# RaduAlexandru/permuto_sdf

Hardware: AMD Instinct MI355X
Metric: ray-samples/sec (encode+MLP+composite) (higher is better)
Workload: dtype f32 (MLP products on 2 fp16 operand pieces per fp32 value, fp32 accumulation; the 3-piece / 24-bit figure is value_fp32_equivalent_24bit)

## Files before the change

### include/psdf.h

```cpp
#ifndef PSDF_H
#define PSDF_H
#include <stdint.h>
#ifdef __cplusplus
extern "C" {
#endif

int64_t psdf_encode_convention(int which);
int psdf_encode_set_conventions(uint32_t hash_multiplier, int rank_tie_raises_later);

int psdf_encode_set_forward_pairs(int pairs);

int psdf_encode_forward(int pos_dim, int nr_feat, int64_t N, int nr_levels, int capacity, const float* positions,
    const float* lattice, const float* scale_factor, const float* shifts, const float* window, int concat_points,
    float points_scaling, float* sliced, void* stream);

int psdf_encode_forward_mark(int pos_dim, int nr_feat, int64_t N, int nr_levels, int capacity, const float* positions,
    const float* lattice, const float* scale_factor, const float* shifts, const float* window, int concat_points,
    float points_scaling, float* sliced, unsigned char* touched_blocks, int block_rows_log2, void* stream);

int psdf_encode_backward(int pos_dim, int nr_feat, int64_t N, int nr_levels, int capacity, const float* positions,
    const float* lattice, const float* scale_factor, const float* shifts, const float* window, int concat_points,
    float points_scaling, const float* grad_sliced, float* grad_lattice, float* grad_positions, void* stream);

int64_t psdf_encode_backward_workspace_bytes(int pos_dim, int nr_feat, int64_t N, int nr_levels, int capacity);
int psdf_encode_backward_ws(int pos_dim, int nr_feat, int64_t N, int nr_levels, int capacity, const float* positions,
    const float* lattice, const float* scale_factor, const float* shifts, const float* window, int concat_points,
    float points_scaling, const float* grad_sliced, float* grad_lattice, float* grad_positions, void* workspace,
    int64_t workspace_bytes, void* stream);
int psdf_encode_backward_level_shares(int* counts, int max_levels);


int psdf_encode_double_backward(int pos_dim, int nr_feat, int64_t N, int nr_levels, int capacity, const float*
    positions, const float* lattice, const float* scale_factor, const float* shifts, const float* window, int
    concat_points, float points_scaling, const float* dd_positions, const float* grad_sliced, float* grad_lattice,
    float* grad_grad_sliced, void* stream);
int psdf_encode_double_backward_ws(int pos_dim, int nr_feat, int64_t N, int nr_levels, int capacity, const float* positions,
                                   const float* lattice, const float* scale_factor, const float* shifts, const float* window,
                                   int concat_points, float points_scaling, const float* dd_positions, const float* grad_sliced,
                                   float* grad_lattice, float* grad_grad_sliced, const float* grad_sliced_direct,
                                   void* workspace, int64_t workspace_bytes, void* stream);

int psdf_mlp_pack_f16(int n_layers, const int* dims, const float* const* weights, const float* const* biases, float* packed,
    void* stream);
int psdf_mlp_forward_f16(int n_layers, const int* dims, int64_t N, const float* X, const float* packed, float* Y, void* stream);

int psdf_mlp_forward_set_form(int waves);
int psdf_mlp_forward_last_form(void);

int psdf_neus_composite_forward(int nr_rays, const int* start_end, int equal, int fixed, int max_nr_samples, const float* sdf,
    const float* dirs, const float* gradients, const float* dt, const float* rgb, const float* inv_s, float cos_anneal_ratio,
    float* pred, float* bg, float* weights, void* stream);
int psdf_neus_composite_backward(int nr_rays, const int* start_end, int equal, int fixed, int max_nr_samples, int max_per_ray,
    const float* grad_pred, const float* grad_bg, const float* sdf, const float* dirs, const float* gradients, const float* dt,
    const float* rgb, const float* inv_s, float cos_anneal_ratio, int reference_compat, float* grad_sdf, float* grad_gradients,
    float* grad_rgb, float* grad_inv_s, void* stream);

int psdf_nerf_composite_forward(int nr_rays, const int* start_end, int equal, int fixed, int max_nr_samples, const float* raw_density,
                                const float* dt, const float* rgb, const float* fg_pred, const float* fg_bg, float* pred_bg,
                                float* pred, void* stream);
int psdf_nerf_composite_backward(int nr_rays, const int* start_end, int equal, int fixed, int max_nr_samples, int max_per_ray,
                                 const float* grad_pred, const float* fg_bg, const float* raw_density, const float* dt,
                                 const float* rgb, int reference_compat, float* grad_raw_density, float* grad_rgb,
// ... 302 lines not shown
```

### permuto_sdf_amd/csrc/encode.hip

```cpp
#include <cstdio>
#include <cstring>
#include <mutex>
#include <type_traits>
#include <vector>

#include "encode_device.h"
#include "encode_plan.h"

namespace {

struct FwdArgs {
  int64_t N;
  int L;
  uint32_t capacity;
  EncConv conv;
  const float *lattice, *scale_factor, *shifts, *window;
  float points_scaling;
  int pad_points;
  float* sliced;
  unsigned char* touched;
  int touch_shift, blocks_per_level;
};

template <int P, int F>
// ... 241 lines not shown
    for (int i = threadIdx.x; i < SC_SLOTS; i += blockDim.x) {
      const uint32_t row = tags[i];
      if (row != SC_EMPTY) {
#pragma unroll
        for (int f = 0; f < F; f++) {
          const float v = sums[i * F + f];
          if (v != 0.f) atomicAdd(table_grad + (int64_t)row * F + f, v);
        }
      }
    }
  }
  static constexpr size_t bytes() { return (size_t)(SC_SLOTS + SC_SLOTS * F + 4) * 4; }
};

template <typename SC>
__device__ __forceinline__ bool cache_vote(SC& sc, int hits, int tries) {
  hits = (int)psdf::wave_sum((float)hits);
  tries = (int)psdf::wave_sum((float)tries);
  if (psdf::lane_id() == 0) {
    atomicAdd(&sc.stats[0], hits);
    atomicAdd(&sc.stats[1], tries);
  }
  __syncthreads();
  return sc.stats[0] * 8 >= sc.stats[1];
}

struct Queues {
  uint16_t* rows;
  float* vals;
  int* tails;
  int cap, np, shift;
};
using psdf::enc_plan::Q_MAX_PARTS;
constexpr int Q_LDS_INTS = 4 * Q_MAX_PARTS + 4;

struct LevelQueues {
  char* rows;
  char* vals;
  uint32_t mask;
};
template <int F>
__device__ __forceinline__ LevelQueues level_queues(const Queues& Q, int level) {
  const int64_t e = (int64_t)level * Q.np * Q.cap;
  return LevelQueues{reinterpret_cast<char*>(Q.rows + e), reinterpret_cast<char*>(Q.vals + e * F), (1u << Q.shift) - 1u};
}
template <int F>
__device__ __forceinline__ void queue_store(const LevelQueues& LQ, uint32_t o, uint32_t row, const float* v) {
  *reinterpret_cast<uint16_t*>(LQ.rows + (o * 2u)) = (uint16_t)(row & LQ.mask);
  if (F == 2) {
    *reinterpret_cast<float2*>(LQ.vals + (o * 8u)) = make_float2(v[0], v[F - 1]);
  } else {
#pragma unroll
    for (int f = 0; f < F; f++) *reinterpret_cast<float*>(LQ.vals + (o * (uint32_t)(F * 4) + (uint32_t)(f * 4))) = v[f];
  }
}

template <int NC, int F>
__device__ __forceinline__ void queue_push(const Queues& Q, int level, int* q_cnt, int* q_base,
                                           const uint32_t (&crow)[NC], const float (&cval)[NC][F],
                                           float* __restrict__ table_grad) {
  int* q_aux = q_base + Q_MAX_PARTS;
  const LevelQueues LQ = level_queues<F>(Q, level);
  if (threadIdx.x < Q.np) q_cnt[threadIdx.x] = 0;
  __syncthreads();
  int slot[NC];
#pragma unroll
  for (int r = 0; r < NC; r++)
    if (crow[r] != Q_NONE) slot[r] = atomicAdd(&q_cnt[crow[r] >> Q.shift], 1);
  __syncthreads();
  if (threadIdx.x < Q.np) {
    const int c = q_cnt[threadIdx.x];
    const int base = c ? atomicAdd(&Q.tails[level * Q.np + threadIdx.x], c) : 0;
    q_base[threadIdx.x] = base;
    q_aux[threadIdx.x] = (int)threadIdx.x * Q.cap + base;
  }
  __syncthreads();
#pragma unroll
  for (int r = 0; r < NC; r++) {
    if (crow[r] == Q_NONE) continue;
    const int part = crow[r] >> Q.shift;
    const int idx = q_base[part] + slot[r];
    if (idx < Q.cap) {
      queue_store<F>(LQ, (uint32_t)(q_aux[part] + slot[r]), crow[r], cval[r]);
    } else {
#pragma unroll
      for (int f = 0; f < F; f++) atomicAdd(table_grad + (int64_t)crow[r] * F + f, cval[r][f]);
    }
  }
}

template <int NC>
__device__ __forceinline__ void queue_push_staged(const Queues& Q, int level, int* q_cnt, int* q_base, int* q_off, int* q_gd,
                                                  float* stage, const uint32_t (&crow)[NC],
                                                  const float (&cval)[NC][2], float* __restrict__ table_grad) {
  uint32_t* st_row = reinterpret_cast<uint32_t*>(stage);
  float2* st_val = reinterpret_cast<float2*>(stage + NC * PSDF_BLOCK);
  const LevelQueues LQ = level_queues<2>(Q, level);
  if (threadIdx.x < Q.np) q_cnt[threadIdx.x] = 0;
  __syncthreads();
  int slot[NC];
#pragma unroll
  for (int r = 0; r < NC; r++)
    if (crow[r] != Q_NONE) slot[r] = atomicAdd(&q_cnt[crow[r] >> Q.shift], 1);
  __syncthreads();
  if (threadIdx.x < 64) {
    const int lane = threadIdx.x;
    const int c = lane < Q.np ? q_cnt[lane] : 0;
    const int incl = psdf::wave_incl_scan_add_i(c);
    if (lane < Q.np) {
      const int base = c ? atomicAdd(&Q.tails[level * Q.np + lane], c) : 0;
      const int off = incl - c;
      q_off[lane] = off;
      q_base[lane] = base - off;
      q_gd[lane] = lane * Q.cap + base - off;
      if (lane == Q.np - 1) q_off[Q.np] = incl;
    }
  }
  __syncthreads();
#pragma unroll
  for (int r = 0; r < NC; r++)
    if (crow[r] != Q_NONE) {
      const int i = q_off[crow[r] >> Q.shift] + slot[r];
      st_row[i] = crow[r];
      st_val[i] = make_float2(cval[r][0], cval[r][1]);
    }
  __syncthreads();
  const int total = q_off[Q.np];
  for (int i = threadIdx.x; i < total; i += PSDF_BLOCK) {
    const uint32_t row = st_row[i];
    const float2 v = st_val[i];
    const int part = row >> Q.shift;
    const int idx = i + q_base[part];
    if (idx < Q.cap) {
      const float vv[2] = {v.x, v.y};
      queue_store<2>(LQ, (uint32_t)(i + q_gd[part]), row, vv);
    } else {
      atomicAdd(table_grad + (int64_t)row * 2, v.x);
      atomicAdd(table_grad + (int64_t)row * 2 + 1, v.y);
    }
  }
}

template <int F, typename SC>
__device__ __forceinline__ void cache_drain_to_queue(SC& sc, const Queues& Q, int level, int* q_cnt,
                                                     int* q_base, float* __restrict__ table_grad) {
  for (int base = 0; base < SC::SC_SLOTS; base += PSDF_BLOCK) {
    const int i = base + threadIdx.x;
    uint32_t crow[1];
    float cval[1][F];
    const uint32_t tag = sc.tags[i];
    static_assert(SC_EMPTY == Q_NONE, "an empty slot is 'no contribution'");
    crow[0] = tag;
#pragma unroll
    for (int f = 0; f < F; f++) cval[0][f] = sc.sums[i * F + f];
    queue_push<1, F>(Q, level, q_cnt, q_base, crow, cval, table_grad);
    sc.tags[i] = SC_EMPTY;
  }
  __syncthreads();
}

struct LevelPlan {
  int n;
  uint32_t gen;
  uint32_t* times;
  uint16_t first[42];
};
template <int P, int F, bool LATTICE, bool POS, bool QUEUE, bool DBL = false>
#if !defined(PSDF_ENC_QWAVES)
#define PSDF_ENC_QWAVES 5
#endif
__global__ void __launch_bounds__(PSDF_BLOCK, QUEUE ? ((P <= 3 && F == 2) ? PSDF_ENC_QWAVES : 4) : 1)
    encode_bwd_kernel(int64_t N, int L, uint32_t capacity, EncConv conv, const float* __restrict__ positions,
                      const float* __restrict__ lattice, const float* __restrict__ scale_factor,
                      const float* __restrict__ shifts, const float* __restrict__ window, float points_scaling,
                      const float* __restrict__ grad_sliced, float* __restrict__ grad_lattice,
                      float* __restrict__ grad_positions, Queues Q, const float* __restrict__ dd_positions = nullptr,
                      float* __restrict__ grad_grad_sliced = nullptr, int pad_points = 0,
                      const float* __restrict__ grad_sliced2 = nullptr, LevelPlan plan = LevelPlan{}) {
  static_assert(!(DBL && POS), "the double backward has no position output");
  extern __shared__ __align__(16) float lds[];
#if defined(PSDF_ENC_PROFILE)
  const long long psdf_prof_t0 = (long long)wall_clock64();
#endif
  int level = blockIdx.y, bx = blockIdx.x, gx = gridDim.x;
  long long plan_t0 = 0;
  if (plan.n) {
    level = 0;
    for (int l = 1; l < plan.n; l++)
      if ((int)blockIdx.x >= (int)plan.first[l]) level = l;
    bx = (int)blockIdx.x - (int)plan.first[level];
    gx = (int)plan.first[level + 1] - (int)plan.first[level];
    plan_t0 = (long long)wall_clock64();
  }
  auto plan_report = [&]() {
    if (plan.n && plan.times && threadIdx.x == 0) {
      long long dt = (long long)wall_clock64() - plan_t0;
      dt = dt < 1 ? 1 : (dt > 0xFFFFFF ? 0xFFFFFF : dt);
      __hip_atomic_store(plan.times + blockIdx.x, ((plan.gen & 255u) << 24) | (uint32_t)dt, __ATOMIC_RELAXED, __HIP_MEMORY_SCOPE_SYSTEM);
    }
  };
  const int64_t ntiles = (N + PSDF_BLOCK - 1) / PSDF_BLOCK;
  if (level >= L) {
    if (DBL) {
      const int e = level - L;
      for (int64_t tile = bx; tile < ntiles; tile += gx) {
        const int64_t n = tile * PSDF_BLOCK + threadIdx.x;
        if (n >= N) continue;
        float u[P];
        load_pos<P>(dd_positions, n, u);
#pragma unroll
        for (int f = 0; f < F; f++) {
          const int d = e * F + f;
          float v = 0.f;
#pragma unroll
          for (int i = 0; i < P; i++)
            if (i == d) v = u[i] * points_scaling;
          if ((d < P || pad_points) && grad_grad_sliced) grad_grad_sliced[((int64_t)level * F + f) * N + n] = v;
        }
      }
    }
    if (POS) {
      const int e = level - L;
      for (int64_t tile = bx; tile < ntiles; tile += gx) {
        const int64_t n = tile * PSDF_BLOCK + threadIdx.x;
        if (n >= N) continue;
#pragma unroll
        for (int f = 0; f < F; f++) {
          const int d = e * F + f;
          if (d < P)
            atomicAdd(grad_positions + n * P + d, grad_sliced[((int64_t)level * F + f) * N + n] * points_scaling);
        }
      }
    }
    plan_report();
    return;
  }
  if (window[level] == 0.f) {
    if (DBL && grad_grad_sliced) {
      for (int64_t tile = bx; tile < ntiles; tile += gx) {
        const int64_t n = tile * PSDF_BLOCK + threadIdx.x;
        if (n >= N) continue;
#pragma unroll
        for (int f = 0; f < F; f++) grad_grad_sliced[((int64_t)level * F + f) * N + n] = 0.f;
      }
    }
    plan_report();
    return;
  }
  using SCache = ScatterCache<F, QUEUE ? 4096 : 8192>;
  SCache sc;
  int* q_cnt = reinterpret_cast<int*>(lds + SCache::bytes() / 4);
  int* q_base = q_cnt + Q_MAX_PARTS;
  int* q_off = q_base + Q_MAX_PARTS;
  int* q_gd = q_off + Q_MAX_PARTS + 1;
  int* q_vote = q_gd + Q_MAX_PARTS;
  if (QUEUE && threadIdx.x < 3) q_vote[threadIdx.x] = 0;
  if (LATTICE) sc.init(lds);
  bool use_cache = LATTICE;
  int hot = 0;
  int hits = 0, tries = 0, iter = 0;
  const float w = window[level];
  const int64_t tbase = (int64_t)level * capacity * F;
  float sfl[P], shl[P];
#pragma unroll
  for (int i = 0; i < P; i++) {
    sfl[i] = scale_factor[level * P + i];
    shl[i] = shifts[level * P + i];
  }
  constexpr int SPT = QUEUE ? QUEUE_SPT : 1;
  constexpr int NC = SPT * (P + 1);
  const int64_t ntiles_w = (N + (int64_t)PSDF_BLOCK * SPT - 1) / ((int64_t)PSDF_BLOCK * SPT);
  for (int64_t tile = bx; tile < ntiles_w; tile += gx, iter++) {
    uint32_t crow[NC];
    float cval[NC][F];
#pragma unroll
    for (int c = 0; c < NC; c++) {
      crow[c] = Q_NONE;
#pragma unroll
      for (int f = 0; f < F; f++) cval[c][f] = 0.f;
    }
#pragma unroll
    for (int sp = 0; sp < SPT; sp++) {
      const int64_t n = (tile * SPT + sp) * PSDF_BLOCK + threadIdx.x;
      if (n < N) {
        float g[F], g2[F];
#pragma unroll
        for (int f = 0; f < F; f++) {
          g[f] = grad_sliced[((int64_t)level * F + f) * N + n];
          g2[f] = (DBL && grad_sliced2) ? grad_sliced2[((int64_t)level * F + f) * N + n] : 0.f;
        }
        float pos[P];
        load_pos<P>(positions, n, pos);
        Simplex<P> s;
// ... 57 lines not shown
#pragma unroll
            for (int f = 0; f < F; f++) dbary[r] = dbary[r] + lattice[tbase + (int64_t)row * F + f] * w * g[f];
          }
        }
        if (DBL && grad_grad_sliced) {
#pragma unroll
          for (int f = 0; f < F; f++) grad_grad_sliced[((int64_t)level * F + f) * N + n] = gg[f];
        }
        if (POS) {
          dbary[P + 1] = dbary[P + 1] + dbary[0];
          float dE[P + 1];
          const float invp = 1.0f / (P + 1);
#pragma unroll
          for (int i = 0; i <= P; i++) {
            float a = 0.f, b = 0.f;
#pragma unroll
            for (int k = 0; k <= P + 1; k++) {
              if (k == P - s.rank[i]) a = dbary[k];
              if (k == P + 1 - s.rank[i]) b = dbary[k];
            }
            dE[i] = (a - b) * invp;
          }
#pragma unroll
          for (int i = 0; i < P; i++) {
            float acc = 0.f;
#pragma unroll
            for (int j = 0; j <= i; j++) acc = acc + dE[j];
            acc = acc - dE[i + 1] * (float)(i + 1);
            atomicAdd(grad_positions + n * P + i, acc * sfl[i]);
          }
        }
      }
    }
    if (LATTICE) {
#pragma unroll
      for (int c = 0; c < NC; c++) {
        const bool own = combine_runs16<F>(crow[c], cval[c]);
        bool absorbed = false;
        if (own && use_cache) {
          const int rc = sc.add(crow[c], cval[c], hot);
          absorbed = rc != 0;
          hits += (rc == 2);
          tries++;
        }
        if (!own || absorbed) crow[c] = Q_NONE;
      }
    }
    if (LATTICE) {
      if (QUEUE) {
        uint32_t all = Q_NONE;
#pragma unroll
        for (int c = 0; c < NC; c++) all &= crow[c];
        const bool any = all != Q_NONE;
        bool go = !use_cache && iter > 0;
        if (!go) {
          const int vw = iter % 3;
          if (threadIdx.x == 0) q_vote[vw == 2 ? 0 : vw + 1] = 0;
          if (__builtin_amdgcn_ballot_w64(any) != 0ull && psdf::lane_id() == 0) q_vote[vw] = 1;
          __syncthreads();
          go = q_vote[vw] != 0;
        }
        if (go) {
          if constexpr (F == 2 && NC * PSDF_BLOCK * 3 * 4 <= SCache::SC_SLOTS * (1 + F) * 4) {
            if (!use_cache && iter > 0)
              queue_push_staged<NC>(Q, level, q_cnt, q_base, q_off, q_gd, lds, crow, cval, grad_lattice + tbase);
            else
              queue_push<NC, F>(Q, level, q_cnt, q_base, crow, cval, grad_lattice + tbase);
          } else {
            queue_push<NC, F>(Q, level, q_cnt, q_base, crow, cval, grad_lattice + tbase);
          }
        }
      } else {
#pragma unroll
        for (int c = 0; c < NC; c++)
          if (crow[c] != Q_NONE) {
#pragma unroll
            for (int f = 0; f < F; f++) atomicAdd(grad_lattice + tbase + (int64_t)crow[c] * F + f, cval[c][f]);
          }
      }
    }
    if (LATTICE && iter == 0) {
      use_cache = cache_vote(sc, hits, tries);
      if (QUEUE && !use_cache) cache_drain_to_queue<F>(sc, Q, level, q_cnt, q_base, grad_lattice + tbase);
    }
  }
  if (LATTICE && !(QUEUE && !use_cache)) sc.flush(grad_lattice + tbase);
  plan_report();
#if defined(PSDF_ENC_PROFILE)
  if (QUEUE && threadIdx.x == 0) {
    const long long dt = (long long)wall_clock64() - psdf_prof_t0;
    int* prof = Q.tails + L * Q.np;
    atomicMax(&prof[level], (int)dt);
    atomicAdd(&prof[64 + level], (int)(dt >> 6));
    atomicAdd(&prof[128 + level], use_cache ? 1 : 0);
  }
#endif
}

template <int P, int F, bool PARTIAL, int POS_LPB>
__global__ void __launch_bounds__(PSDF_BLOCK)
    encode_bwd_pos_kernel(int64_t N, int L, int Lt, uint32_t capacity, EncConv conv, const float* __restrict__ positions,
                          const float* __restrict__ lattice, const float* __restrict__ scale_factor,
                          const float* __restrict__ shifts, const float* __restrict__ window, float points_scaling,
                          int pad_points, const float* __restrict__ grad_sliced, const unsigned char* __restrict__ skip,
                          float* __restrict__ grad_positions) {
  const int64_t n = (int64_t)blockIdx.x * PSDF_BLOCK + threadIdx.x;
  if (n >= N) return;
  if (skip && skip[n]) return;
  float pos[P];
  load_pos<P>(positions, n, pos);
  float gp[P];
#pragma unroll
  for (int i = 0; i < P; i++) gp[i] = 0.f;
#pragma unroll
  for (int li = 0; li < POS_LPB; li++) {
    const int level = blockIdx.y * POS_LPB + li;
    if (level >= Lt) break;
    float g[F];
#pragma unroll
    for (int f = 0; f < F; f++)
// ... 400 lines not shown
    launch_bwd_pos_lpb<P, F, 4>(c, grad_sliced, skip, grad_positions, true);
  else if (c.N >= ((int64_t)1 << 17))
    launch_bwd_pos_lpb<P, F, 2>(c, grad_sliced, skip, grad_positions, false);
  else
    launch_bwd_pos_lpb<P, F, 8>(c, grad_sliced, skip, grad_positions, false);
  return PSDF_OK;
}

plan::QueuePlan queue_plan(int pos_dim, int nr_feat, int64_t N, int nr_levels, int capacity) {
  static const int64_t min_n = plan::env_long("PSDF_ENC_QUEUE_MIN_N", (int64_t)1 << 13);
  static const int delta = env_int("PSDF_ENC_QUEUE_SLICE_LOG2_DELTA", 1);
  return plan::queue_plan(pos_dim, nr_feat, N, nr_levels, capacity, min_n, delta);
}
Queues queue_carve(void* ws, const plan::QueuePlan& p) {
  char* b = (char*)ws;
  return Queues{(uint16_t*)b, (float*)(b + p.rows_bytes), (int*)(b + p.rows_bytes + p.vals_bytes), p.cap, p.np, p.shift};
}
bool queue_begin(int pos_dim, int nr_feat, const EncCall& c, bool wanted, void* ws, int64_t ws_bytes, size_t also_zeroed, Queues& Q,
                 hipError_t& e) {
  const plan::QueuePlan p = (wanted && ws) ? queue_plan(pos_dim, nr_feat, c.N, c.nr_levels, c.capacity) : plan::QueuePlan{};
  if (p.bytes == 0 || ws_bytes < p.bytes) return false;
  Q = queue_carve(ws, p);
  e = hipMemsetAsync(Q.tails, 0, (size_t)c.nr_levels * Q.np * sizeof(int) + also_zeroed, c.stream);
  return true;
}

struct EncBalance {
  int levels = 0, total = 0, kind = 0, bucket = -1;
  const void* ident = nullptr;
  uint32_t gen = 0;
  uint64_t last_use = 0;
  std::vector<int> counts;
  uint32_t* times[2] = {nullptr, nullptr};
  int device = -1;
};
constexpr int BAL_STATES = 16;
std::mutex g_shares_mu;
std::vector<int> g_last_shares;

bool encode_balance(int nr_levels, int64_t N, int total, int64_t super_tiles, LevelPlan& lp, const void* ident, int kind) {
  static const bool off = env_int("PSDF_ENC_BWD_BALANCE", 1) == 0;
  static std::mutex mu;
  static EncBalance states[BAL_STATES];
  static uint64_t tick = 0;
  if (!plan::deal_eligible(off, nr_levels, total, N)) return false;
  std::lock_guard<std::mutex> lock(mu);
  const int bucket = plan::size_bucket(N);
  int device = -1;
  (void)hipGetDevice(&device);
  EncBalance* Bp = nullptr;
  for (auto& st_ : states)
    if (st_.times[0] && st_.ident == ident && st_.device == device && st_.kind == kind && st_.levels == nr_levels && st_.bucket == bucket &&
        st_.total == total)
      Bp = &st_;
  if (!Bp) {
    for (auto& st_ : states)
      if (!Bp || st_.last_use < Bp->last_use) Bp = &st_;
    if (!Bp->times[0]) {
      for (int i = 0; i < 2; i++) {
        void* h = nullptr;
        if (hipHostMalloc(&h, plan::BAL_MAX_WG * sizeof(uint32_t), hipHostMallocMapped) != hipSuccess || !h) {
          (void)hipGetLastError();
          if (i == 1) (void)hipHostFree(Bp->times[0]);
          Bp->times[0] = Bp->times[1] = nullptr;
          return false;
        }
        Bp->times[i] = (uint32_t*)h;
      }
    }
    memset(Bp->times[0], 0, plan::BAL_MAX_WG * sizeof(uint32_t));
    memset(Bp->times[1], 0, plan::BAL_MAX_WG * sizeof(uint32_t));
    Bp->levels = 0;
  }
  EncBalance& B = *Bp;
  B.last_use = ++tick;
  if (!B.times[0] || !B.times[1]) return false;
  const int cap = (int)(super_tiles < total ? super_tiles : total);
  if (B.levels != nr_levels || (int)B.counts.size() != nr_levels) {
    B.levels = nr_levels;
    B.kind = kind;
    B.ident = ident;
    B.device = device;
    B.bucket = bucket;
    B.total = total;
    B.counts = plan::first_deal(nr_levels, total);
  } else {
    plan::redeal_from_times(B.counts, B.times[B.gen & 1], B.gen, total, cap);
  }
  B.gen++;
  lp.n = nr_levels;
  lp.gen = B.gen;
  lp.times = B.times[B.gen & 1];
  const int at = plan::deal_layout(B.counts, cap, lp.first);
  std::lock_guard<std::mutex> l2(g_shares_mu);
  g_last_shares = B.counts;
  return at <= plan::BAL_MAX_WG;
}

template <class Kernel>
unsigned resident_round(Kernel kern, size_t shm, const EncCall& c, int deal_levels, int kind, LevelPlan& deal) {
  int per_cu = 0;
  const bool known = hipOccupancyMaxActiveBlocksPerMultiprocessor(&per_cu, kern, PSDF_BLOCK, shm) == hipSuccess && per_cu > 0;
  if (!known) (void)hipGetLastError();
  const int resident = known ? per_cu * device_cus() : 0;
  const int64_t tiles = plan::super_tiles(c.N, PSDF_BLOCK * QUEUE_SPT);
  deal = LevelPlan{};
  if (known && deal_levels > 0 && !encode_balance(deal_levels, c.N, resident, tiles, deal, c.lattice, kind)) deal = LevelPlan{};
  return plan::round_share(resident, c.nr_levels, tiles);
}

template <int F>
constexpr size_t binning_shm() { return ScatterCache<F, 4096>::bytes() + Q_LDS_INTS * sizeof(int); }

template <int P, int F, bool DBL>
unsigned launch_binning(const EncCall& c, int levels, const float* grad_sliced, float* grad_lattice, const Queues& Q,
                        const float* dd_positions, float* grad_grad_sliced, const float* grad_sliced2) {
  const auto kern = encode_bwd_kernel<P, F, true, false, true, DBL>;
  LevelPlan deal;
  const unsigned gx = resident_round(kern, binning_shm<F>(), c, levels, DBL ? 1 : 0, deal);
  launch_enc(kern, deal.n ? dim3(deal.first[deal.n]) : dim3(gx, levels), binning_shm<F>(), c, grad_sliced, grad_lattice,
             (float*)nullptr, Q, dd_positions, grad_grad_sliced, DBL ? c.pad : 0, grad_sliced2, deal);
  return gx;
}

template <int F>
int launch_queue_reduce(const EncCall& c, const Queues& Q, float* grad_lattice) {
  const size_t lds_b = (size_t)(1 << Q.shift) * F * sizeof(float);
  const hipError_t e =
      hipFuncSetAttribute((const void*)encode_bwd_reduce_kernel<F>, hipFuncAttributeMaxDynamicSharedMemorySize, (int)lds_b);
  if (e != hipSuccess) return (int)e;
  hipLaunchKernelGGL((encode_bwd_reduce_kernel<F>), dim3(Q.np, c.nr_levels), dim3(1024), lds_b, c.stream, (uint32_t)c.capacity, Q,
                     grad_lattice);
  return PSDF_OK;
}

#if defined(PSDF_ENC_PROFILE)
void enc_profile_report(const EncCall& c, int pos_dim, const Queues& Q, unsigned gx) {
  static int calls = 0;
  if (++calls != 8) return;
  (void)hipStreamSynchronize(c.stream);
  int prof[192];
  (void)hipMemcpy(prof, Q.tails + c.nr_levels * Q.np, sizeof(prof), hipMemcpyDeviceToHost);
  std::vector<int> tails((size_t)c.nr_levels * Q.np);
  (void)hipMemcpy(tails.data(), Q.tails, tails.size() * sizeof(int), hipMemcpyDeviceToHost);
  for (int l = 0; l < c.nr_levels; l++) {
    long long queued = 0;
    for (int q = 0; q < Q.np; q++) queued += tails[(size_t)l * Q.np + q];
    fprintf(stderr, "[enc-profile] level %2d: max %8d ticks, mean %8.0f ticks, cache kept by %d of %u workgroups, queued %lld of %lld "
            "contributions (%.1f %%)\n", l, prof[l], 64.0 * prof[64 + l] / gx, prof[128 + l], gx, queued,
            (long long)c.N * (pos_dim + 1), 100.0 * queued / ((double)c.N * (pos_dim + 1)));
  }
}
#endif

bool pos_fused() {
  static const bool on = env_int("PSDF_ENC_POS_FUSED", 0) != 0;
  return on;
}

template <int P, int F>
int launch_bwd(int_c<P> p, int_c<F> f, const EncCall& c, const float* grad_sliced, float* grad_lattice, float* grad_positions,
               const Queues* Q) {
  const float* const no_in = nullptr;
  float* const no_out = nullptr;
  constexpr size_t plain_shm = ScatterCache<F, 8192>::bytes() + Q_LDS_INTS * sizeof(int);
  if (!grad_lattice) return launch_bwd_pos(p, f, c, grad_sliced, nullptr, grad_positions);
  if (!Q) {
    if (grad_positions)
      launch_enc(encode_bwd_kernel<P, F, true, true, false>, plain_grid(c), plain_shm, c, grad_sliced, grad_lattice, grad_positions,
                 Queues{}, no_in, no_out, 0, no_in, LevelPlan{});
    else
      launch_enc(encode_bwd_kernel<P, F, true, false, false>, plain_grid(c), plain_shm, c, grad_sliced, grad_lattice, grad_positions,
                 Queues{}, no_in, no_out, 0, no_in, LevelPlan{});
    return PSDF_OK;
  }
  [[maybe_unused]] unsigned gx;
  if (grad_positions && pos_fused()) {
    const auto kern = encode_bwd_kernel<P, F, true, true, true>;
    LevelPlan none;
    gx = resident_round(kern, binning_shm<F>(), c, 0, 0, none);
    launch_enc(kern, dim3(gx, c.Lt), binning_shm<F>(), c, grad_sliced, grad_lattice, grad_positions, *Q, no_in, no_out, 0, no_in, none);
  } else {
    gx = launch_binning<P, F, false>(c, c.nr_levels, grad_sliced, grad_lattice, *Q, no_in, no_out, no_in);
    if (grad_positions) launch_bwd_pos(p, f, c, grad_sliced, nullptr, grad_positions);
  }
  const int rc = launch_queue_reduce<F>(c, *Q, grad_lattice);
#if defined(PSDF_ENC_PROFILE)
  if (rc == PSDF_OK) enc_profile_report(c, P, *Q, gx);
#endif
  return rc;
}

template <int P, int F>
int launch_dbl_queue(int_c<P>, int_c<F>, const EncCall& c, const float* dd_positions, const float* grad_sliced, float* grad_lattice,
                     float* grad_grad_sliced, const float* grad_sliced_direct, const Queues& Q) {
  launch_binning<P, F, true>(c, c.Lt, grad_sliced, grad_lattice, Q, dd_positions, grad_grad_sliced, grad_sliced_direct);
  return launch_queue_reduce<F>(c, Q, grad_lattice);
}

template <int P, int F>
int launch_dbl_plain(int_c<P>, int_c<F>, const EncCall& c, const float* dd_positions, const float* grad_sliced, float* grad_lattice,
                     float* grad_grad_sliced) {
  if (grad_lattice)
    launch_enc(encode_dbl_bwd_kernel<P, F, true>, plain_grid(c), ScatterCache<F>::bytes(), c, c.pad, dd_positions, grad_sliced,
               grad_lattice, grad_grad_sliced);
  else
    launch_enc(encode_dbl_bwd_kernel<P, F, false>, plain_grid(c), 0, c, c.pad, dd_positions, grad_sliced, grad_lattice,
               grad_grad_sliced);
  return PSDF_OK;
}

}

// ... 25 lines not shown
int psdf_encode_forward(int pos_dim, int nr_feat, int64_t N, int nr_levels, int capacity, const float* positions,
                        const float* lattice, const float* scale_factor, const float* shifts, const float* window,
                        int concat_points, float points_scaling, float* sliced, void* stream) {
  return encode_forward_impl(pos_dim, nr_feat, N, nr_levels, capacity, positions, lattice, scale_factor, shifts, window,
                             concat_points, points_scaling, nullptr, sliced, stream);
}

int psdf_encode_forward_masked(int pos_dim, int nr_feat, int64_t N, int nr_levels, int capacity, const float* positions,
                               const float* lattice, const float* scale_factor, const float* shifts, const float* window,
                               int concat_points, float points_scaling, const unsigned char* skip, float* sliced,
                               void* stream) {
  return encode_forward_impl(pos_dim, nr_feat, N, nr_levels, capacity, positions, lattice, scale_factor, shifts, window,
                             concat_points, points_scaling, skip, sliced, stream);
}

int psdf_encode_forward_mark(int pos_dim, int nr_feat, int64_t N, int nr_levels, int capacity, const float* positions,
                             const float* lattice, const float* scale_factor, const float* shifts, const float* window,
                             int concat_points, float points_scaling, float* sliced, unsigned char* touched_blocks,
                             int block_rows_log2, void* stream) {
  if (!touched_blocks || block_rows_log2 < 0 || block_rows_log2 > 20) return PSDF_ERR_ARG;
  return encode_forward_impl(pos_dim, nr_feat, N, nr_levels, capacity, positions, lattice, scale_factor, shifts, window,
                             concat_points, points_scaling, nullptr, sliced, stream, touched_blocks, block_rows_log2);
}

int64_t psdf_encode_backward_workspace_bytes(int pos_dim, int nr_feat, int64_t N, int nr_levels, int capacity) {
  return queue_plan(pos_dim, nr_feat, N, nr_levels, capacity).bytes;
}

int psdf_encode_backward_level_shares(int* counts, int max_levels) {
  std::lock_guard<std::mutex> lock(g_shares_mu);
  const int n = (int)g_last_shares.size();
  for (int l = 0; l < n && l < max_levels; l++) counts[l] = g_last_shares[l];
  return n;
}

int psdf_encode_backward_ws(int pos_dim, int nr_feat, int64_t N, int nr_levels, int capacity, const float* positions,
                            const float* lattice, const float* scale_factor, const float* shifts, const float* window,
                            int concat_points, float points_scaling, const float* grad_sliced, float* grad_lattice,
                            float* grad_positions, void* workspace, int64_t workspace_bytes, void* stream) {
  EncCall c;
  if (N == 0 || (!grad_lattice && !grad_positions)) return PSDF_OK;
  if (!enc_call(c, pos_dim, nr_feat, N, nr_levels, capacity, positions, lattice, scale_factor, shifts, window, concat_points,
                points_scaling, stream) || !grad_sliced)
    return PSDF_ERR_ARG;
  if (!grad_positions) c.Lt = nr_levels;
  Queues Q{};
  hipError_t e = hipSuccess;
#if defined(PSDF_ENC_PROFILE)
  const size_t profile_slots = 1024;
#else
  const size_t profile_slots = 0;
#endif
  const bool use_queue = queue_begin(pos_dim, nr_feat, c, grad_lattice, workspace, workspace_bytes, profile_slots, Q, e);
  if (e != hipSuccess) return (int)e;
  const int rc = dispatch_pf(pos_dim, nr_feat, [&](auto p, auto f) {
    return launch_bwd(p, f, c, grad_sliced, grad_lattice, grad_positions, use_queue ? &Q : nullptr);
  });
  if (rc == PSDF_OK) psdf::g_last_path[psdf::PATH_ENCODE_BWD] = use_queue ? 2 : (grad_lattice ? 1 : 3);
  return launched(rc);
}

int psdf_encode_backward(int pos_dim, int nr_feat, int64_t N, int nr_levels, int capacity, const float* positions,
                         const float* lattice, const float* scale_factor, const float* shifts, const float* window,
                         int concat_points, float points_scaling, const float* grad_sliced, float* grad_lattice,
                         float* grad_positions, void* stream) {
  return psdf_encode_backward_ws(pos_dim, nr_feat, N, nr_levels, capacity, positions, lattice, scale_factor, shifts,
// ... 66 lines not shown
```

### permuto_sdf_amd/csrc/encode_plan.h

```cpp
#pragma once
#include <cstdint>
#include <cstdlib>
#include <vector>

namespace psdf {
namespace enc_plan {

inline int env_int(const char* name, int dflt) { const char* v = getenv(name); return v ? atoi(v) : dflt; }
inline long long env_long(const char* name, long long dflt) { const char* v = getenv(name); return v ? atoll(v) : dflt; }

constexpr int Q_MAX_PARTS = 64;

struct QueuePlan {
  int cap, np, shift;
  int64_t rows_bytes, vals_bytes, tails_bytes, bytes;
};

inline QueuePlan queue_plan(int pos_dim, int nr_feat, int64_t N, int nr_levels, int capacity, int64_t min_n, int slice_delta) {
  if (N < min_n) return QueuePlan{};
  const int base = (nr_feat <= 2) ? 14 : (nr_feat <= 4 ? 13 : 12);
  int shift = base - (slice_delta < 0 ? 0 : (slice_delta > 3 ? 3 : slice_delta));
  while (shift < base && ((capacity + (1 << shift) - 1) >> shift) > Q_MAX_PARTS) shift++;
  const int rpp = 1 << shift;
  const int np = (capacity + rpp - 1) / rpp;
// ... 50 lines not shown
    for (int l = 1; l < n; l++)
      if (counts[l] > counts[big]) big = l;
    if (counts[big] <= BAL_MIN_PER_LEVEL) break;
    counts[big]--;
    used--;
  }
}

inline bool redeal_from_times(std::vector<int>& counts, const volatile uint32_t* times, uint32_t gen, int total, int cap) {
  std::vector<double> work(counts.size(), 0.0);
  int id = 0;
  for (size_t l = 0; l < counts.size(); l++)
    for (int b = 0; b < counts[l]; b++, id++) {
      const uint32_t v = times[id];
      if ((v >> 24) != (gen & 255u) || (v & 0xFFFFFFu) == 0u) return false;
      work[l] += (double)(v & 0xFFFFFFu);
    }
  redeal(counts, work.data(), total, cap);
  return true;
}

inline int deal_layout(std::vector<int>& counts, int cap, uint16_t* first) {
  int at = 0;
  for (size_t l = 0; l < counts.size(); l++) {
    if (counts[l] > cap) counts[l] = cap;
    if (counts[l] < 1) counts[l] = 1;
    first[l] = (uint16_t)at;
    at += counts[l];
  }
  first[counts.size()] = (uint16_t)at;
  return at;
}

constexpr int FWD_MAX_SLOTS = 42;
constexpr uint8_t FWD_SLOT_NONE = 0xFF;
struct FwdSlots {
  int n;
  uint8_t a[FWD_MAX_SLOTS];
  uint8_t b[FWD_MAX_SLOTS];
};

inline FwdSlots forward_slots(int L, int Lt, int pairs) {
  FwdSlots s{};
  if (L < 1 || Lt < L || Lt >= (int)FWD_SLOT_NONE) return s;
  if (pairs < 0) pairs = 0;
  if (pairs > L / 2) pairs = L / 2;
  if (Lt - pairs > FWD_MAX_SLOTS) return s;
  int at = 0;
  for (int i = 0; i < pairs; i++, at++) {
    s.a[at] = (uint8_t)i;
    s.b[at] = (uint8_t)(L - 1 - i);
  }
  for (int l = pairs; l < Lt; l++) {
    if (l < L && l >= L - pairs) continue;
    s.a[at] = (uint8_t)l;
    s.b[at] = FWD_SLOT_NONE;
    at++;
  }
  s.n = at;
  return s;
}

inline int forward_pairs_default(int L, int64_t N) {
  (void)N;
  return L / 2;
}
// ... 4 lines not shown
```

### permuto_sdf_amd/encoding.py

```python
import math

import numpy as np
import torch

from . import _lib as L
from . import conventions as CV


def scale_factor_tensor(scale_list, pos_dim):
    scale_list = np.asarray(scale_list, dtype=np.float64)
    sf = np.empty((len(scale_list), pos_dim), dtype=np.float64)
    for i in range(pos_dim):
        sf[:, i] = 1.0 / (CV.scale_term(i, pos_dim) * scale_list)
    return torch.from_numpy(sf.astype(np.float32))


class _Cfg:

    def __init__(self, pos_dim, capacity, nr_levels, nr_feat, concat_points, points_scaling, concat_layout=None):
        self.pos_dim, self.capacity, self.nr_levels, self.nr_feat = pos_dim, capacity, nr_levels, nr_feat
        self.concat_points, self.points_scaling = bool(concat_points), float(points_scaling)
        self.concat_mode = CV.concat_mode(concat_points, concat_layout)
        self.extra = int(math.ceil(pos_dim / nr_feat)) if concat_points else 0
        self.channels = CV.channels(pos_dim, nr_levels, nr_feat, self.concat_mode)
# ... 7 lines not shown
    return (L.c_i(int(cfg.concat_mode)), L.c_f(cfg.points_scaling))


def encode_forward_raw(cfg, positions, lattice, scale_factor, shifts, window, skip=None, out=None, touched=None,
                       block_rows_log2=7):
    L.require_cuda(positions, lattice)
    N = positions.shape[0]
    sliced = out if out is not None else torch.empty((cfg.channels, N), dtype=torch.float32, device=positions.device)
    if touched is not None and skip is None:
        L.call("psdf_encode_forward_mark", *_head(cfg, N), L.ptr(positions), L.ptr(lattice), L.ptr(scale_factor),
               L.ptr(shifts), L.ptr(window), *_tail(cfg), L.ptr(sliced), L.ptr(touched), L.c_i(block_rows_log2), L.stream())
    elif skip is None:
        L.call("psdf_encode_forward", *_head(cfg, N), L.ptr(positions), L.ptr(lattice), L.ptr(scale_factor),
               L.ptr(shifts), L.ptr(window), *_tail(cfg), L.ptr(sliced), L.stream())
    else:
        L.call("psdf_encode_forward_masked", *_head(cfg, N), L.ptr(positions), L.ptr(lattice), L.ptr(scale_factor),
               L.ptr(shifts), L.ptr(window), *_tail(cfg), L.ptr(skip), L.ptr(sliced), L.stream())
    return sliced


def encode_backward_raw(cfg, positions, lattice, scale_factor, shifts, window, g_fm, g_lat, g_pos):
    import ctypes
    N = positions.shape[0]
    ws, nbytes = None, 0
    if g_lat is not None:
        fn = L.lib().psdf_encode_backward_workspace_bytes
        fn.restype = ctypes.c_int64
        nbytes = int(fn(L.c_i(cfg.pos_dim), L.c_i(cfg.nr_feat), L.c_l(N), L.c_i(cfg.nr_levels), L.c_i(cfg.capacity)))
        if nbytes > 0:
            ws = torch.empty(nbytes, dtype=torch.uint8, device=positions.device)
    L.call("psdf_encode_backward_ws", *_head(cfg, N), L.ptr(positions), L.ptr(lattice), L.ptr(scale_factor),
           L.ptr(shifts), L.ptr(window), *_tail(cfg), L.ptr(g_fm), L.ptr(g_lat), L.ptr(g_pos), L.ptr(ws), L.c_l(nbytes),
           L.stream())


def _backward_workspace(cfg, N, device):
    import ctypes
    fn = L.lib().psdf_encode_backward_workspace_bytes
    fn.restype = ctypes.c_int64
    nbytes = int(fn(L.c_i(cfg.pos_dim), L.c_i(cfg.nr_feat), L.c_l(N), L.c_i(cfg.nr_levels), L.c_i(cfg.capacity)))
    return (torch.empty(nbytes, dtype=torch.uint8, device=device) if nbytes > 0 else None), nbytes


def encode_double_backward_raw(cfg, positions, lattice, scale_factor, shifts, window, dd_positions, g_fm, g_lat, gg_fm,
                               direct_fm=None):
    N = positions.shape[0]
    ws, nbytes = _backward_workspace(cfg, N, positions.device) if g_lat is not None else (None, 0)
    L.call("psdf_encode_double_backward_ws", *_head(cfg, N), L.ptr(positions), L.ptr(lattice), L.ptr(scale_factor), L.ptr(shifts),
           L.ptr(window), *_tail(cfg), L.ptr(dd_positions), L.ptr(g_fm), L.ptr(g_lat), L.ptr(gg_fm), L.ptr(direct_fm), L.ptr(ws),
           L.c_l(nbytes), L.stream())


def morton_order(positions, lo=None, hi=None):
    p = positions.detach().float()
    lo = p.min(0).values if lo is None else lo
    hi = p.max(0).values if hi is None else hi
    q = ((p - lo) / (hi - lo).clamp_min(1e-20) * 1023.0).clamp(0, 1023).to(torch.int64)
    code = torch.zeros(p.shape[0], dtype=torch.int64, device=p.device)
    for b in range(10):
        for a in range(p.shape[1]):
            code |= ((q[:, a] >> b) & 1) << (p.shape[1] * b + a)
    return torch.argsort(code)


def _feature_major(g):
    gt = g.t()
# ... 218 lines not shown
```

Baseline: 1.023 billion.

## Choose per-level backward scatter mode adaptively from in-kernel observations

Each workgroup in the encoder backward kernel now reports observations: whether its cache held, whether the queue overflowed, and its owner, point and hit counts. The host uses these to decide per level whether to skip the LDS scatter cache and the run-combining step, pushing straight to the queues instead. A full probe run is forced every 16 calls, and a level that overflows falls back to probing. This removes cache init, voting and draining on levels with low reuse, at the cost of a feedback loop that depends on stale observations and extra mapped host memory. The metric is a forward throughput, so this backward-only change may not affect it.

```diff
diff --git a/include/psdf.h b/include/psdf.h
--- a/include/psdf.h
+++ b/include/psdf.h
@@ -28,6 +28,11 @@
     float points_scaling, const float* grad_sliced, float* grad_lattice, float* grad_positions, void* workspace,
     int64_t workspace_bytes, void* stream);
 int psdf_encode_backward_level_shares(int* counts, int max_levels);
+int psdf_encode_backward_level_modes(int* modes, int max_levels);
+int psdf_encode_backward_level_reports(int pos_dim, int64_t* reports, int max_levels);
+int psdf_encode_backward_probe_every(void);
+int psdf_encode_set_backward_mode(int mode);
+int psdf_encode_set_backward_level_mode(int level, int mode);
 
 
 int psdf_encode_double_backward(int pos_dim, int nr_feat, int64_t N, int nr_levels, int capacity, const float*
diff --git a/permuto_sdf_amd/csrc/encode.hip b/permuto_sdf_amd/csrc/encode.hip
--- a/permuto_sdf_amd/csrc/encode.hip
+++ b/permuto_sdf_amd/csrc/encode.hip
@@ -297,7 +297,7 @@
   int cap, np, shift;
 };
 using psdf::enc_plan::Q_MAX_PARTS;
-constexpr int Q_LDS_INTS = 4 * Q_MAX_PARTS + 4;
+constexpr int Q_LDS_INTS = 4 * Q_MAX_PARTS + 8;
 
 struct LevelQueues {
   char* rows;
@@ -321,7 +321,7 @@
 }
 
 template <int NC, int F>
-__device__ __forceinline__ void queue_push(const Queues& Q, int level, int* q_cnt, int* q_base,
+__device__ __forceinline__ void queue_push(const Queues& Q, int level, int* q_cnt, int* q_base, int* q_over,
                                            const uint32_t (&crow)[NC], const float (&cval)[NC][F],
                                            float* __restrict__ table_grad) {
   int* q_aux = q_base + Q_MAX_PARTS;
@@ -348,6 +348,7 @@
     if (idx < Q.cap) {
       queue_store<F>(LQ, (uint32_t)(q_aux[part] + slot[r]), crow[r], cval[r]);
     } else {
+      *q_over = 1;
 #pragma unroll
       for (int f = 0; f < F; f++) atomicAdd(table_grad + (int64_t)crow[r] * F + f, cval[r][f]);
     }
@@ -356,7 +357,7 @@
 
 template <int NC>
 __device__ __forceinline__ void queue_push_staged(const Queues& Q, int level, int* q_cnt, int* q_base, int* q_off, int* q_gd,
-                                                  float* stage, const uint32_t (&crow)[NC],
+                                                  int* q_over, float* stage, const uint32_t (&crow)[NC],
                                                   const float (&cval)[NC][2], float* __restrict__ table_grad) {
   uint32_t* st_row = reinterpret_cast<uint32_t*>(stage);
   float2* st_val = reinterpret_cast<float2*>(stage + NC * PSDF_BLOCK);
@@ -400,6 +401,7 @@
       const float vv[2] = {v.x, v.y};
       queue_store<2>(LQ, (uint32_t)(i + q_gd[part]), row, vv);
     } else {
+      *q_over = 1;
       atomicAdd(table_grad + (int64_t)row * 2, v.x);
       atomicAdd(table_grad + (int64_t)row * 2 + 1, v.y);
     }
@@ -408,7 +410,7 @@
 
 template <int F, typename SC>
 __device__ __forceinline__ void cache_drain_to_queue(SC& sc, const Queues& Q, int level, int* q_cnt,
-                                                     int* q_base, float* __restrict__ table_grad) {
+                                                     int* q_base, int* q_over, float* __restrict__ table_grad) {
   for (int base = 0; base < SC::SC_SLOTS; base += PSDF_BLOCK) {
     const int i = base + threadIdx.x;
     uint32_t crow[1];
@@ -418,7 +420,7 @@
     crow[0] = tag;
 #pragma unroll
     for (int f = 0; f < F; f++) cval[0][f] = sc.sums[i * F + f];
-    queue_push<1, F>(Q, level, q_cnt, q_base, crow, cval, table_grad);
+    queue_push<1, F>(Q, level, q_cnt, q_base, q_over, crow, cval, table_grad);
     sc.tags[i] = SC_EMPTY;
   }
   __syncthreads();
@@ -428,6 +430,8 @@
   int n;
   uint32_t gen;
   uint32_t* times;
+  uint32_t* obs;
+  uint32_t modes[psdf::enc_plan::MODE_WORDS];
   uint16_t first[42];
 };
 template <int P, int F, bool LATTICE, bool POS, bool QUEUE, bool DBL = false>
@@ -457,13 +461,20 @@
     gx = (int)plan.first[level + 1] - (int)plan.first[level];
     plan_t0 = (long long)wall_clock64();
   }
-  auto plan_report = [&]() {
+  namespace ep = psdf::enc_plan;
+  auto plan_report = [&](uint32_t observed, uint32_t hits = 0u) {
     if (plan.n && plan.times && threadIdx.x == 0) {
       long long dt = (long long)wall_clock64() - plan_t0;
       dt = dt < 1 ? 1 : (dt > 0xFFFFFF ? 0xFFFFFF : dt);
       __hip_atomic_store(plan.times + blockIdx.x, ((plan.gen & 255u) << 24) | (uint32_t)dt, __ATOMIC_RELAXED, __HIP_MEMORY_SCOPE_SYSTEM);
+      if (plan.obs) {
+        static_assert(ep::OBS_WORDS == 2, "two words per workgroup");
+        __hip_atomic_store(plan.obs + 2 * blockIdx.x, observed, __ATOMIC_RELAXED, __HIP_MEMORY_SCOPE_SYSTEM);
+        __hip_atomic_store(plan.obs + 2 * blockIdx.x + 1, ep::obs_hits_word(plan.gen, hits), __ATOMIC_RELAXED, __HIP_MEMORY_SCOPE_SYSTEM);
+      }
     }
   };
+  const uint32_t nothing_observed = ep::obs_word(plan.gen, true, false, ep::OBS_NO_OWNERS, 0);
   const int64_t ntiles = (N + PSDF_BLOCK - 1) / PSDF_BLOCK;
   if (level >= L) {
     if (DBL) {
@@ -497,7 +508,7 @@
         }
       }
     }
-    plan_report();
+    plan_report(nothing_observed);
     return;
   }
   if (window[level] == 0.f) {
@@ -509,7 +520,7 @@
         for (int f = 0; f < F; f++) grad_grad_sliced[((int64_t)level * F + f) * N + n] = 0.f;
       }
     }
-    plan_report();
+    plan_report(nothing_observed);
     return;
   }
   using SCache = ScatterCache<F, QUEUE ? 4096 : 8192>;
@@ -519,11 +530,15 @@
   int* q_off = q_base + Q_MAX_PARTS;
   int* q_gd = q_off + Q_MAX_PARTS + 1;
   int* q_vote = q_gd + Q_MAX_PARTS;
-  if (QUEUE && threadIdx.x < 3) q_vote[threadIdx.x] = 0;
-  if (LATTICE) sc.init(lds);
-  bool use_cache = LATTICE;
+  int* q_over = q_vote + 3;
+  const int mode = (QUEUE && LATTICE && plan.n) ? ep::unpack_mode(plan.modes, level) : ep::MODE_PROBE;
+  const bool queue_only = mode == ep::MODE_QUEUE || mode == ep::MODE_QUEUE_RAW;
+  const bool combine = mode != ep::MODE_QUEUE_RAW;
+  if (QUEUE && threadIdx.x < 4) q_vote[threadIdx.x] = 0;
+  if (LATTICE && !queue_only) sc.init(lds);
+  bool use_cache = LATTICE && !queue_only;
   int hot = 0;
-  int hits = 0, tries = 0, iter = 0;
+  int hits = 0, tries = 0, iter = queue_only ? 1 : 0;
   const float w = window[level];
   const int64_t tbase = (int64_t)level * capacity * F;
   float sfl[P], shl[P];
@@ -647,7 +662,7 @@
         }
       }
     }
-    if (LATTICE) {
+    if (LATTICE && combine) {
 #pragma unroll
       for (int c = 0; c < NC; c++) {
         const bool own = combine_runs16<F>(crow[c], cval[c]);
@@ -678,11 +693,11 @@
         if (go) {
           if constexpr (F == 2 && NC * PSDF_BLOCK * 3 * 4 <= SCache::SC_SLOTS * (1 + F) * 4) {
             if (!use_cache && iter > 0)
-              queue_push_staged<NC>(Q, level, q_cnt, q_base, q_off, q_gd, lds, crow, cval, grad_lattice + tbase);
+              queue_push_staged<NC>(Q, level, q_cnt, q_base, q_off, q_gd, q_over, lds, crow, cval, grad_lattice + tbase);
             else
-              queue_push<NC, F>(Q, level, q_cnt, q_base, crow, cval, grad_lattice + tbase);
+              queue_push<NC, F>(Q, level, q_cnt, q_base, q_over, crow, cval, grad_lattice + tbase);
           } else {
-            queue_push<NC, F>(Q, level, q_cnt, q_base, crow, cval, grad_lattice + tbase);
+            queue_push<NC, F>(Q, level, q_cnt, q_base, q_over, crow, cval, grad_lattice + tbase);
           }
         }
       } else {
@@ -696,11 +711,25 @@
     }
     if (LATTICE && iter == 0) {
       use_cache = cache_vote(sc, hits, tries);
-      if (QUEUE && !use_cache) cache_drain_to_queue<F>(sc, Q, level, q_cnt, q_base, grad_lattice + tbase);
+      if (QUEUE && !use_cache) cache_drain_to_queue<F>(sc, Q, level, q_cnt, q_base, q_over, grad_lattice + tbase);
     }
   }
   if (LATTICE && !(QUEUE && !use_cache)) sc.flush(grad_lattice + tbase);
-  plan_report();
+  uint32_t observed = 0u, observed_hits = 0u;
+  if (QUEUE && LATTICE && plan.n && plan.obs) {
+    __syncthreads();
+    const bool over = *q_over != 0;
+    if (queue_only) {
+      observed = ep::obs_word(plan.gen, false, over, ep::OBS_NO_OWNERS, 0);
+    } else {
+      static_assert(PSDF_BLOCK * SPT <= (int)ep::OBS_MAX_POINTS && PSDF_BLOCK * NC < (int)ep::OBS_NO_OWNERS, "obs_word fields");
+      const int64_t rest = N - (int64_t)bx * (PSDF_BLOCK * SPT);
+      const uint32_t points = (uint32_t)(rest < PSDF_BLOCK * SPT ? rest : PSDF_BLOCK * SPT);
+      observed = ep::obs_word(plan.gen, use_cache, over, (uint32_t)sc.stats[1], points);
+      observed_hits = (uint32_t)sc.stats[0];
+    }
+  }
+  plan_report(observed, observed_hits);
 #if defined(PSDF_ENC_PROFILE)
   if (QUEUE && threadIdx.x == 0) {
     const long long dt = (long long)wall_clock64() - psdf_prof_t0;
@@ -1167,13 +1196,29 @@
   uint64_t last_use = 0;
   std::vector<int> counts;
   uint32_t* times[2] = {nullptr, nullptr};
+  uint32_t* obs[2] = {nullptr, nullptr};
+  std::vector<uint8_t> decided, launched;
+  std::vector<uint8_t> barred;
+  long long calls = 0;
   int device = -1;
 };
 constexpr int BAL_STATES = 16;
+constexpr int BAL_WORDS = 1 + plan::OBS_WORDS;
 std::mutex g_shares_mu;
 std::vector<int> g_last_shares;
-
-bool encode_balance(int nr_levels, int64_t N, int total, int64_t super_tiles, LevelPlan& lp, const void* ident, int kind) {
+std::vector<uint8_t> g_last_modes;
+const uint32_t *g_last_obs = nullptr, *g_last_times = nullptr;
+uint32_t g_last_gen = 0;
+int g_mode_all = -1;
+int g_mode_level[plan::BAL_MAX_LEVELS];
+bool g_mode_level_set = false;
+int forced_mode(int level) {
+  if (g_mode_level_set && level < plan::BAL_MAX_LEVELS && g_mode_level[level] >= 0) return g_mode_level[level];
+  return g_mode_all;
+}
+
+bool encode_balance(int nr_levels, int64_t N, int total, int64_t super_tiles, LevelPlan& lp, const void* ident, int kind,
+                    int contribs_per_point) {
   static const bool off = env_int("PSDF_ENC_BWD_BALANCE", 1) == 0;
   static std::mutex mu;
   static EncBalance states[BAL_STATES];
@@ -1194,17 +1239,18 @@
     if (!Bp->times[0]) {
       for (int i = 0; i < 2; i++) {
         void* h = nullptr;
-        if (hipHostMalloc(&h, plan::BAL_MAX_WG * sizeof(uint32_t), hipHostMallocMapped) != hipSuccess || !h) {
+        if (hipHostMalloc(&h, BAL_WORDS * plan::BAL_MAX_WG * sizeof(uint32_t), hipHostMallocMapped) != hipSuccess || !h) {
           (void)hipGetLastError();
           if (i == 1) (void)hipHostFree(Bp->times[0]);
-          Bp->times[0] = Bp->times[1] = nullptr;
+          Bp->times[0] = Bp->times[1] = Bp->obs[0] = Bp->obs[1] = nullptr;
           return false;
         }
         Bp->times[i] = (uint32_t*)h;
-      }
-    }
-    memset(Bp->times[0], 0, plan::BAL_MAX_WG * sizeof(uint32_t));
-    memset(Bp->times[1], 0, plan::BAL_MAX_WG * sizeof(uint32_t));
+        Bp->obs[i] = (uint32_t*)h + plan::BAL_MAX_WG;
+      }
+    }
+    memset(Bp->times[0], 0, BAL_WORDS * plan::BAL_MAX_WG * sizeof(uint32_t));
+    memset(Bp->times[1], 0, BAL_WORDS * plan::BAL_MAX_WG * sizeof(uint32_t));
     Bp->levels = 0;
   }
   EncBalance& B = *Bp;
@@ -1219,28 +1265,46 @@
     B.bucket = bucket;
     B.total = total;
     B.counts = plan::first_deal(nr_levels, total);
+    B.decided.assign((size_t)nr_levels, (uint8_t)plan::MODE_PROBE);
+    B.launched = B.barred = B.decided;
+    B.calls = 0;
   } else {
+    plan::update_modes(B.decided, B.launched, B.counts, B.obs[B.gen & 1], B.gen, contribs_per_point, &B.barred);
     plan::redeal_from_times(B.counts, B.times[B.gen & 1], B.gen, total, cap);
   }
   B.gen++;
   lp.n = nr_levels;
   lp.gen = B.gen;
   lp.times = B.times[B.gen & 1];
+  lp.obs = B.obs[B.gen & 1];
   const int at = plan::deal_layout(B.counts, cap, lp.first);
+  const bool probe = plan::probe_call(B.calls++, plan::MODE_PROBE_EVERY);
+  if (probe) B.barred.assign((size_t)nr_levels, 0);
   std::lock_guard<std::mutex> l2(g_shares_mu);
+  for (int l = 0; l < nr_levels; l++) {
+    const int forced = forced_mode(l);
+    B.launched[l] = (uint8_t)(forced >= 0 ? forced : (probe ? plan::MODE_PROBE : B.decided[l]));
+  }
+  plan::pack_modes(B.launched, lp.modes);
   g_last_shares = B.counts;
+  g_last_modes = B.launched;
+  g_last_obs = lp.obs;
+  g_last_times = lp.times;
+  g_last_gen = B.gen;
+  if (at > plan::BAL_MAX_WG) g_last_modes.clear();
   return at <= plan::BAL_MAX_WG;
 }
 
 template <class Kernel>
-unsigned resident_round(Kernel kern, size_t shm, const EncCall& c, int deal_levels, int kind, LevelPlan& deal) {
+unsigned resident_round(Kernel kern, size_t shm, const EncCall& c, int deal_levels, int kind, int contribs_per_point, LevelPlan& deal) {
   int per_cu = 0;
   const bool known = hipOccupancyMaxActiveBlocksPerMultiprocessor(&per_cu, kern, PSDF_BLOCK, shm) == hipSuccess && per_cu > 0;
   if (!known) (void)hipGetLastError();
   const int resident = known ? per_cu * device_cus() : 0;
   const int64_t tiles = plan::super_tiles(c.N, PSDF_BLOCK * QUEUE_SPT);
   deal = LevelPlan{};
-  if (known && deal_levels > 0 && !encode_balance(deal_levels, c.N, resident, tiles, deal, c.lattice, kind)) deal = LevelPlan{};
+  if (known && deal_levels > 0 && !encode_balance(deal_levels, c.N, resident, tiles, deal, c.lattice, kind, contribs_per_point))
+    deal = LevelPlan{};
   return plan::round_share(resident, c.nr_levels, tiles);
 }
 
@@ -1252,7 +1316,7 @@
                         const float* dd_positions, float* grad_grad_sliced, const float* grad_sliced2) {
   const auto kern = encode_bwd_kernel<P, F, true, false, true, DBL>;
   LevelPlan deal;
-  const unsigned gx = resident_round(kern, binning_shm<F>(), c, levels, DBL ? 1 : 0, deal);
+  const unsigned gx = resident_round(kern, binning_shm<F>(), c, levels, DBL ? 1 : 0, P + 1, deal);
   launch_enc(kern, deal.n ? dim3(deal.first[deal.n]) : dim3(gx, levels), binning_shm<F>(), c, grad_sliced, grad_lattice,
              (float*)nullptr, Q, dd_positions, grad_grad_sliced, DBL ? c.pad : 0, grad_sliced2, deal);
   return gx;
@@ -1313,7 +1377,7 @@
   if (grad_positions && pos_fused()) {
     const auto kern = encode_bwd_kernel<P, F, true, true, true>;
     LevelPlan none;
-    gx = resident_round(kern, binning_shm<F>(), c, 0, 0, none);
+    gx = resident_round(kern, binning_shm<F>(), c, 0, 0, P + 1, none);
     launch_enc(kern, dim3(gx, c.Lt), binning_shm<F>(), c, grad_sliced, grad_lattice, grad_positions, *Q, no_in, no_out, 0, no_in, none);
   } else {
     gx = launch_binning<P, F, false>(c, c.nr_levels, grad_sliced, grad_lattice, *Q, no_in, no_out, no_in);
@@ -1405,6 +1469,60 @@
   const int n = (int)g_last_shares.size();
   for (int l = 0; l < n && l < max_levels; l++) counts[l] = g_last_shares[l];
   return n;
+}
+
+int psdf_encode_backward_level_modes(int* modes, int max_levels) {
+  std::lock_guard<std::mutex> lock(g_shares_mu);
+  const int n = (int)g_last_modes.size();
+  for (int l = 0; l < n && l < max_levels; l++) modes[l] = g_last_modes[l];
+  return n;
+}
+
+int psdf_encode_backward_level_reports(int pos_dim, int64_t* reports, int max_levels) {
+  std::lock_guard<std::mutex> lock(g_shares_mu);
+  const int n = (int)g_last_modes.size();
+  if (n == 0 || !g_last_obs || (int)g_last_shares.size() != n) return 0;
+  int id = 0;
+  for (int l = 0; l < n; id += g_last_shares[l], l++) {
+    const plan::LevelReport r = plan::level_report(g_last_obs + (size_t)plan::OBS_WORDS * id, g_last_shares[l], g_last_gen);
+    if (!r.complete) return -1;
+    if (l >= max_levels) continue;
+    int64_t* out = reports + 7 * l;
+    out[0] = r.held;
+    out[1] = r.overflowed;
+    out[2] = r.owners;
+    out[3] = r.points * (pos_dim + 1);
+    out[6] = r.hits;
+    out[4] = out[5] = 0;
+    for (int b = 0; b < g_last_shares[l]; b++) {
+      const int64_t t = (int64_t)(((const volatile uint32_t*)g_last_times)[id + b] & 0xFFFFFFu);
+      out[4] += t;
+      out[5] = t > out[5] ? t : out[5];
+    }
+  }
+  return n;
+}
+
+int psdf_encode_backward_probe_every(void) { return plan::MODE_PROBE_EVERY; }
+
+int psdf_encode_set_backward_mode(int mode) {
+  if (mode < -1 || mode > plan::MODE_CACHE) return PSDF_ERR_ARG;
+  if (mode == plan::MODE_CACHE) return PSDF_ERR_UNSUPPORTED;
+  std::lock_guard<std::mutex> lock(g_shares_mu);
+  g_mode_all = mode;
+  return PSDF_OK;
+}
+
+int psdf_encode_set_backward_level_mode(int level, int mode) {
+  if (level < 0 || level >= plan::BAL_MAX_LEVELS || mode < -1 || mode > plan::MODE_CACHE) return PSDF_ERR_ARG;
+  if (mode == plan::MODE_CACHE) return PSDF_ERR_UNSUPPORTED;
+  std::lock_guard<std::mutex> lock(g_shares_mu);
+  if (!g_mode_level_set) {
+    for (int& m : g_mode_level) m = -1;
+    g_mode_level_set = true;
+  }
+  g_mode_level[level] = mode;
+  return PSDF_OK;
 }
 
 int psdf_encode_backward_ws(int pos_dim, int nr_feat, int64_t N, int nr_levels, int capacity, const float* positions,
diff --git a/permuto_sdf_amd/csrc/encode_plan.h b/permuto_sdf_amd/csrc/encode_plan.h
--- a/permuto_sdf_amd/csrc/encode_plan.h
+++ b/permuto_sdf_amd/csrc/encode_plan.h
@@ -106,6 +106,80 @@
   return at;
 }
 
+constexpr int MODE_PROBE = 0, MODE_QUEUE = 1, MODE_QUEUE_RAW = 2, MODE_CACHE = 3;
+constexpr int MODE_WORDS = 3;
+constexpr int MODE_PROBE_EVERY = 16;
+
+constexpr int OBS_WORDS = 2;
+constexpr uint32_t OBS_HOLD = 1u << 23, OBS_OVERFLOW = 1u << 22, OBS_NO_OWNERS = 0xFFFu, OBS_MAX_POINTS = 0x3FFu;
+constexpr uint32_t obs_word(uint32_t gen, bool hold, bool overflow, uint32_t owners, uint32_t points) {
+  return ((gen & 255u) << 24) | (hold ? OBS_HOLD : 0u) | (overflow ? OBS_OVERFLOW : 0u) | ((owners & 0xFFFu) << 10) |
+         (points & OBS_MAX_POINTS);
+}
+constexpr uint32_t obs_hits_word(uint32_t gen, uint32_t hits) { return ((gen & 255u) << 24) | (hits & 0xFFFFFFu); }
+
+struct LevelReport {
+  bool complete;
+  int held, overflowed, unobserved;
+  long long owners, points, hits;
+};
+inline LevelReport level_report(const volatile uint32_t* obs, int count, uint32_t gen) {
+  LevelReport r{true, 0, 0, 0, 0, 0, 0};
+  for (int b = 0; b < count; b++) {
+    const uint32_t v = obs[OBS_WORDS * b], h = obs[OBS_WORDS * b + 1];
+    if (v == 0u || (v >> 24) != (gen & 255u) || (h >> 24) != (gen & 255u)) {
+      r.complete = false;
+      continue;
+    }
+    r.held += (v & OBS_HOLD) != 0u;
+    r.overflowed += (v & OBS_OVERFLOW) != 0u;
+    const uint32_t owners = (v >> 10) & 0xFFFu;
+    if (owners == OBS_NO_OWNERS) {
+      r.unobserved++;
+    } else {
+      r.owners += owners;
+      r.points += v & OBS_MAX_POINTS;
+      r.hits += h & 0xFFFFFFu;
+    }
+  }
+  return r;
+}
+
+constexpr int MODE_REUSE_DEN = 4;
+inline int next_mode(const LevelReport& r, int launched, int decided, int contribs_per_point) {
+  if (!r.complete) return decided;
+  if (r.overflowed > 0) return MODE_PROBE;
+  if (launched != MODE_PROBE) return decided;
+  if (r.unobserved > 0 || r.points <= 0) return MODE_PROBE;
+  if (r.held > 0) return r.hits * MODE_REUSE_DEN < r.owners ? MODE_QUEUE : MODE_PROBE;
+  (void)contribs_per_point;
+  return MODE_QUEUE;
+}
+
+inline void update_modes(std::vector<uint8_t>& decided, const std::vector<uint8_t>& launched, const std::vector<int>& counts,
+                         const volatile uint32_t* obs, uint32_t gen, int contribs_per_point, std::vector<uint8_t>* barred = nullptr) {
+  int id = 0;
+  for (size_t l = 0; l < counts.size(); id += counts[l], l++) {
+    if (l >= decided.size() || l >= launched.size()) continue;
+    const LevelReport r = level_report(obs + (size_t)OBS_WORDS * id, counts[l], gen);
+    decided[l] = (uint8_t)next_mode(r, launched[l], decided[l], contribs_per_point);
+    if (barred && l < barred->size()) {
+      if (r.complete && r.overflowed > 0 && launched[l] != MODE_PROBE) (*barred)[l] = 1;
+      if ((*barred)[l]) decided[l] = (uint8_t)MODE_PROBE;
+    }
+  }
+}
+
+inline bool probe_call(long long call, int every) { return every <= 1 || call % every == 0; }
+
+inline void pack_modes(const std::vector<uint8_t>& modes, uint32_t (&words)[MODE_WORDS]) {
+  for (int w = 0; w < MODE_WORDS; w++) words[w] = 0u;
+  for (size_t l = 0; l < modes.size() && l < (size_t)16 * MODE_WORDS; l++) words[l >> 4] |= (uint32_t)(modes[l] & 3u) << ((l & 15) * 2);
+}
+constexpr int unpack_mode(const uint32_t* words, int level) {
+  return level < 16 * MODE_WORDS ? (int)((words[level >> 4] >> ((level & 15) * 2)) & 3u) : MODE_PROBE;
+}
+
 constexpr int FWD_MAX_SLOTS = 42;
 constexpr uint8_t FWD_SLOT_NONE = 0xFF;
 struct FwdSlots {
diff --git a/permuto_sdf_amd/encoding.py b/permuto_sdf_amd/encoding.py
--- a/permuto_sdf_amd/encoding.py
+++ b/permuto_sdf_amd/encoding.py
@@ -63,6 +63,34 @@
     L.call("psdf_encode_backward_ws", *_head(cfg, N), L.ptr(positions), L.ptr(lattice), L.ptr(scale_factor),
            L.ptr(shifts), L.ptr(window), *_tail(cfg), L.ptr(g_fm), L.ptr(g_lat), L.ptr(g_pos), L.ptr(ws), L.c_l(nbytes),
            L.stream())
+
+
+def set_backward_mode(mode):
+    L.call("psdf_encode_set_backward_mode", L.c_i(mode))
+
+
+def set_backward_level_mode(level, mode):
+    L.call("psdf_encode_set_backward_level_mode", L.c_i(level), L.c_i(mode))
+
+
+def backward_level_modes():
+    import ctypes
+    fn = L.lib().psdf_encode_backward_level_modes
+    fn.restype = ctypes.c_int
+    buf = (ctypes.c_int * 64)()
+    return list(buf[:fn(buf, 64)])
+
+
+def backward_level_reports(pos_dim):
+    import ctypes
+    fn = L.lib().psdf_encode_backward_level_reports
+    fn.restype = ctypes.c_int
+    buf = (ctypes.c_int64 * (7 * 64))()
+    n = fn(L.c_i(pos_dim), buf, 64)
+    if n <= 0:
+        return None
+    keys = ("held", "overflowed", "owners", "contributions", "ticks", "max_ticks", "hits")
+    return [dict(zip(keys, buf[7 * l:7 * l + 7])) for l in range(n)]
 
 
 def _backward_workspace(cfg, N, device):
```

Result: no change. 1.028 billion (median of 3 runs) (+0.5%).
